# VealFang/PLI-SLAM

Hardware: AMD Instinct MI355X
Metric: stereo frames/sec (ORB+LSD extract+match), 752x480 EuRoC (higher is better)
Workload: dtype u8; 1 GPU; 1xMI355X: 752x480 stereo pairs, extract + stereo Hamming match (BASELINE configs[1] shape, batched); 752x480, 1200 ORB kp (8 levels x1.2) + LSD/LBD (<=100 lines); 256 stereo frames per GPU per step; frames_per_gpu=256, parallelism=frame-batch data parallel, 1 rank(s), gather of result tables to rank 0

## Files before the change

### pli_slam_amd/csrc/common.hpp

```cpp
#pragma once
#include <hip/hip_runtime.h>
#include <cstdint>
#include <cstdio>
#include <cstring>
#include <string>
#include <vector>
#include <map>
#include "../../include/pli_frontend.h"

namespace pli {

constexpr int MAX_LEVELS = 16;
constexpr int CELL_CAP = 512;
constexpr int GRID_COLS = 64;
constexpr int GRID_ROWS = 48;
constexpr int LSD_CHUNK = 4096;

struct LevelGeom {
  int w, h, pitch;
  int64_t offset;
  int minBX, minBY, maxBX, maxBY;
  int nCols, nRows, wCell, hCell;
  int cellBase;
  int nfeatures;
// ... 52 lines not shown
  int races;
  int pad4[31];
};
constexpr int RX_ARENA_BITS = 40;

struct RxSeed {
  int rank, xy;
  float ang, sx, sy;
};

constexpr int RX_QCAP = 16;
constexpr int RX_HAND = RX_QCAP - 8;

struct RxRect {
  int rank, off, cnt;
  float sumdx, sumdy;
  int approx;
};

struct TxDirtyLists {
  int2* list;
  int* cnt;
  const int* order;
  int ts, ntx, nty, W;
  int64_t npix;
  int rmask = -1;
  const int* perm = nullptr;
  int xcdAffine = 0;
  int stamp = 0;
};

constexpr int LSD_ID_INF = 0x7FFFFFFF;
constexpr int TX_EMIT_CAP = 16384;
struct ZeroRanges {
  uint32_t* p[12];
  int64_t words[12];
};

struct TxKeys {
  const double* mg;
  const unsigned long long* maxMg;
  double rho;
  int nBins, pixbits;
  int* idPlane;
  float4* recPack = nullptr;
  int lazyMargin = 8;
  int2* hot = nullptr;
  const float2* cold = nullptr;
  int pack = 0;
};

struct TxTailArgs {
  const DevParams* Pp;
  RxCtl* ctl;
  const float4* rec;
  int2* own;
  const int2* list;
  const int* tileCnt;
  int ts, ntx, nty;
  int* rgSize;
  int2* rgBox;
  int* rgDirty;
  int* tileAct;
  int* tileTouch;
  int TW, TH;
  int* arena;
// ... 37 lines not shown
```

### pli_slam_amd/csrc/kernels.hpp

```cpp
#pragma once
#include "common.hpp"

namespace pli {

struct BlurPlane {
  int w, h, pitchIn, pitchOut;
  int64_t offIn, offOut;
  int tilesX, tileBase;
};
struct BlurJob {
  int nplanes;
  BlurPlane pl[MAX_LEVELS];
  int k[7];
  int radius;
};
struct LbdCoef { float L[21]; float G[63]; };

constexpr signed char ORB_PATTERN_HOST[1024] = {
#include "../../include/pli_orb_pattern.inc"
};
constexpr int orbPatternReach() {
  int best = 0;
  for (int i = 0; i < 512; ++i) {
    const long long x = ORB_PATTERN_HOST[2 * i], y = ORB_PATTERN_HOST[2 * i + 1], r2 = x * x + y * y;
// ... 89 lines not shown
__global__ void k_tri_match(const pli_keypoint* __restrict__ kp1, const uint8_t* __restrict__ desc1, const int* __restrict__ node1, const uint8_t* __restrict__ hasMp1, const uint8_t* __restrict__ stereo1, int n1, const int* __restrict__ kfOff, const pli_keypoint* __restrict__ kfKp, const uint8_t* __restrict__ kfDesc, const uint8_t* __restrict__ kfStereo, const uint32_t* __restrict__ sNode, const uint16_t* __restrict__ sIdx, const int* __restrict__ nListed, const float* __restrict__ F12, const float* __restrict__ ep, const float* __restrict__ scaleFactor, const float* __restrict__ sigma2, int onlyStereo, int coarse, int checkOri, int* __restrict__ matches12, int* __restrict__ stat);
__global__ void k_tri_finish(const pli_keypoint* __restrict__ kp1, int n1, const int* __restrict__ kfOff, const pli_keypoint* __restrict__ kfKp, int* __restrict__ matches12, int* __restrict__ stat);
__global__ void k_kb8_rays(const pli_keypoint* __restrict__ kp1, int n1, int n1Left, const pli_keypoint* __restrict__ kfKp, const int* __restrict__ kfOff, const int* __restrict__ kfNleft, int nkf, Kb8 camL, Kb8 camR, float2* __restrict__ ray1, float2* __restrict__ kfRay);
__global__ void k_tri_match_kb8(const pli_keypoint* __restrict__ kp1, const uint8_t* __restrict__ desc1, const int* __restrict__ node1, const uint8_t* __restrict__ hasMp1, const float2* __restrict__ ray1, int n1, int n1Left, const int* __restrict__ kfOff, const int* __restrict__ kfNleft, const pli_keypoint* __restrict__ kfKp, const uint8_t* __restrict__ kfDesc, const float2* __restrict__ kfRay, const uint32_t* __restrict__ sNode, const uint16_t* __restrict__ sIdx, const int* __restrict__ nListed, const float* __restrict__ rel, Kb8 camL, Kb8 camR, const float* __restrict__ sigma2, int coarse, int checkOri, int* __restrict__ matches12, int* __restrict__ stat);
__global__ void k_search_by_bow_kf(const uint8_t* __restrict__ desc1, const float* __restrict__ angle1, const int* __restrict__ node1, const uint8_t* __restrict__ valid1, int n1, const int* __restrict__ kfOff, const uint8_t* __restrict__ kfDesc, const float* __restrict__ kfAngle, const uint32_t* __restrict__ sNode, const uint16_t* __restrict__ sIdx, const int* __restrict__ nListed, int keyCap, float nnratio, int checkOri, int* __restrict__ matches12, int* __restrict__ nmatchesOut);
struct FuseSurvivor { int kf, mp; float u, v, ur, radius; int level, pad; };
__global__ void k_fuse_grid(const int* __restrict__ kfOff, const pli_keypoint* __restrict__ kfKp, pli_fuse_camera cam, int* __restrict__ cellStart, uint16_t* __restrict__ sIdx);
__global__ void k_fuse_project(const pli_fuse_point* __restrict__ mp, int nmp, int nkf, const float* __restrict__ kfPose, const uint8_t* __restrict__ skip, pli_fuse_camera cam, float th, const float* __restrict__ levelRatio, int nlevels, const float* __restrict__ scaleFactor, FuseSurvivor* __restrict__ surv, int* __restrict__ nSurv, int* __restrict__ bestIdx, int* __restrict__ bestDist);
template <int G> __global__ void k_fuse_match(const FuseSurvivor* __restrict__ surv, const int* __restrict__ nSurv, int nmp, const uint8_t* __restrict__ mpDesc, const int* __restrict__ kfOff, const pli_keypoint* __restrict__ kfKp, const uint8_t* __restrict__ kfDesc, const float* __restrict__ kfUright, const int* __restrict__ cellStart, const uint16_t* __restrict__ sIdx, pli_fuse_camera cam, const float* __restrict__ invSigma2, int reprojGate, int* __restrict__ bestIdx, int* __restrict__ bestDist);
__global__ void k_sim3_project(const pli_fuse_point* __restrict__ mp, int nmp, int npair, const float* __restrict__ kfPose, const uint8_t* __restrict__ skip, pli_fuse_camera cam, float th, const float* __restrict__ levelRatio, int nlevels, const float* __restrict__ scaleFactor, int form, FuseSurvivor* __restrict__ surv, int* __restrict__ candCount, int* __restrict__ bestIdx);
__global__ void k_sim3_candidates(const FuseSurvivor* __restrict__ surv, int64_t nslot, const uint8_t* __restrict__ mpDesc, const int* __restrict__ kfOff, const pli_keypoint* __restrict__ kfKp, const uint8_t* __restrict__ kfDesc, const int* __restrict__ cellStart, const uint16_t* __restrict__ sIdx, pli_fuse_camera cam, int distLimit, int width, unsigned long long* __restrict__ candKeys, int* __restrict__ candCount);
__global__ void k_sim3_assign(const FuseSurvivor* __restrict__ surv, int nmp, const uint8_t* __restrict__ mpDesc, const int* __restrict__ kfOff, const pli_keypoint* __restrict__ kfKp, const uint8_t* __restrict__ kfDesc, const uint8_t* __restrict__ occupied, const int* __restrict__ cellStart, const uint16_t* __restrict__ sIdx, pli_fuse_camera cam, int distLimit, int width, const unsigned long long* __restrict__ candKeys, const int* __restrict__ candCount, int* __restrict__ rowPoint, int* __restrict__ bestIdx, int* __restrict__ nmatchesOut);
__global__ void k_reloc_project(const pli_fuse_point* __restrict__ mp, const int* __restrict__ mpOff, int ncand, const float* __restrict__ pose, pli_fuse_camera cam, float th, const float* __restrict__ levelRatio, int nlevels, const float* __restrict__ scaleFactor, FuseSurvivor* __restrict__ surv, int* __restrict__ candCount, int* __restrict__ bestIdx);
__global__ void k_reloc_candidates(const FuseSurvivor* __restrict__ surv, int64_t nslot, const uint8_t* __restrict__ mpDesc, const int* __restrict__ fOff, const pli_keypoint* __restrict__ fKp, const uint8_t* __restrict__ fDesc, const int* __restrict__ cellStart, const uint16_t* __restrict__ sIdx, pli_fuse_camera cam, int distLimit, int width, unsigned long long* __restrict__ candKeys, int* __restrict__ candCount);
__global__ void k_reloc_assign(const FuseSurvivor* __restrict__ surv, const int* __restrict__ mpOff, const uint8_t* __restrict__ mpDesc, const float* __restrict__ mpAngle, const int* __restrict__ fOff, const pli_keypoint* __restrict__ fKp, const uint8_t* __restrict__ fDesc, int nf, const uint8_t* __restrict__ occupied, const int* __restrict__ cellStart, const uint16_t* __restrict__ sIdx, pli_fuse_camera cam, int distLimit, int width, int checkOri, const unsigned long long* __restrict__ candKeys, const int* __restrict__ candCount, int* __restrict__ rowPoint, int* __restrict__ bestIdx, int* __restrict__ nmatchesOut);
__global__ void k_init_candidates(const pli_keypoint* __restrict__ kp1, const uint8_t* __restrict__ desc1, int n1, const float* __restrict__ prevMatched, const pli_keypoint* __restrict__ kp2, const uint8_t* __restrict__ desc2, const int* __restrict__ cellStart, const uint16_t* __restrict__ sIdx, pli_fuse_camera cam, float radius, int distLimit, int width, unsigned long long* __restrict__ candKeys, int* __restrict__ candCount);
__global__ void k_init_assign(const pli_keypoint* __restrict__ kp1, const uint8_t* __restrict__ desc1, int n1, const float* __restrict__ prevMatched, const pli_keypoint* __restrict__ kp2, const uint8_t* __restrict__ desc2, int n2, const int* __restrict__ cellStart, const uint16_t* __restrict__ sIdx, pli_fuse_camera cam, float radius, int distLimit, int width, float nnratio, int checkOri, const unsigned long long* __restrict__ candKeys, const int* __restrict__ candCount, int* __restrict__ matches12, int* __restrict__ raw12, int* __restrict__ nmatchesOut);
__global__ void k_fisheye_triangulate(const pli_keypoint* __restrict__ kpL, const pli_keypoint* __restrict__ kpR, const int* __restrict__ knnIdx, const int* __restrict__ knnDist, int nl, int nr, int monoL, int monoR, Kb8 c1, Kb8 c2, const float* __restrict__ R12t12, const float* __restrict__ sigma2, int* __restrict__ l2r, int* __restrict__ r2l, float* __restrict__ depth, float* __restrict__ p3d, int* __restrict__ nmatches);
__global__ void k_fill_f32(float* __restrict__ dst, int n, float v);
__global__ void k_proj_assign_fisheye(const pli_proj_query* __restrict__ qL, const pli_proj_query* __restrict__ qR, const uint8_t* __restrict__ qdesc, int nq, const pli_keypoint* __restrict__ kpL, const uint8_t* __restrict__ descL, const uint8_t* __restrict__ occL, const int* __restrict__ l2r, int nL, const pli_keypoint* __restrict__ kpR, const uint8_t* __restrict__ descR, const uint8_t* __restrict__ occR, const int* __restrict__ r2l, int nR, const float* __restrict__ noUright, float minX, float maxX, float minY, float maxY, float nnratio, const unsigned long long* __restrict__ keysL, const int* __restrict__ cntL, const unsigned long long* __restrict__ keysR, const int* __restrict__ cntR, int* __restrict__ mpL, int* __restrict__ mpR, int* __restrict__ nmatchesOut);
__global__ void k_proj2_candidates(const pli_proj_query* __restrict__ q, const uint8_t* __restrict__ qdesc, int nq, const pli_keypoint* __restrict__ kpL, const uint8_t* __restrict__ descL, int nL, const pli_keypoint* __restrict__ kpR, const uint8_t* __restrict__ descR, int nR, const float* __restrict__ noUright, float minX, float maxX, float minY, float maxY, unsigned long long* __restrict__ candKeys, int* __restrict__ candCount, int* __restrict__ leftOpen);
__global__ void k_proj2_assign(const pli_proj_query* __restrict__ q, const uint8_t* __restrict__ qdesc, int nq, const pli_keypoint* __restrict__ kpL, const uint8_t* __restrict__ descL, const uint8_t* __restrict__ occL, int nL, const pli_keypoint* __restrict__ kpR, const uint8_t* __restrict__ descR, const uint8_t* __restrict__ occR, int nR, const float* __restrict__ noUright, float minX, float maxX, float minY, float maxY, int checkOri, const unsigned long long* __restrict__ candKeys, const int* __restrict__ candCount, const int* __restrict__ leftOpen, int* __restrict__ rawIdx2, int* __restrict__ hist, int* __restrict__ accepts);
__global__ void k_proj2_finish(const pli_proj_query* __restrict__ q, int nq, const pli_keypoint* __restrict__ kpL, const pli_keypoint* __restrict__ kpR, int checkOri, const int* __restrict__ rawIdx2, const int* __restrict__ hist, const int* __restrict__ accepts, int* __restrict__ bestIdx2, int* __restrict__ nmatchesOut);
__global__ void k_lapping_order(const pli_keypoint* __restrict__ srcKp, const uint8_t* __restrict__ srcDesc, int n, float lap0, float lap1, pli_keypoint* __restrict__ dstKp, uint8_t* __restrict__ dstDesc, int* __restrict__ monoCount);

__global__ void k_tx_tail(TxTailArgs A);
__global__ void k_tx_rec_from_hot(const RxCtl* __restrict__ ctl, const int2* __restrict__ hotAll, const float2* __restrict__ coldAll, float4* __restrict__ recAll, int64_t npix, int img0);
__global__ void k_tx_hot_trig_err(unsigned long long* __restrict__ maxErrBits);
__global__ void k_tx_cells(RxCtl* __restrict__ ctl, const int* __restrict__ stampAll, int* __restrict__ tileTouchAll, int ncell, int nimg, int img0, int t, int mode, int* __restrict__ list, int* __restrict__ cnt);
__global__ void k_tx_diffmark_cells(RxCtl* __restrict__ ctl, const int2* __restrict__ ownAll, const int* __restrict__ rankAll, const int2* __restrict__ rgBoxAll, int* __restrict__ rgDirtyAll, int* __restrict__ tileActAll, int W, int H, int TW, int TH, int t, int img0, const int* __restrict__ rgLostAll, TxDirtyLists DL, const int* __restrict__ list, const int* __restrict__ cnt);
__global__ void k_tx_prep_cells(const RxCtl* __restrict__ ctl, int2* __restrict__ ownAll, const int* __restrict__ rankAll, const int* __restrict__ rgDirtyAll, int W, int H, int TW, int TH, int t, int img0, int rmask, const int* __restrict__ list, const int* __restrict__ cnt, int stamp);
__global__ void k_zero_ranges(ZeroRanges Z);
__global__ void k_tx_collect(RxCtl* __restrict__ ctl, const int* __restrict__ idPlaneAll, const int2* __restrict__ ownAll, const int* __restrict__ rgSizeAll, int64_t npix, int minReg, int* __restrict__ candAll, int* __restrict__ candCnt, int img0, int emitCap);
__global__ void k_tx_emit_sorted(const RxCtl* __restrict__ ctl, const int* __restrict__ candAll, const int* __restrict__ candCnt, const float4* __restrict__ rgSegAll, int64_t npix, int rmask, float* __restrict__ segAll, int* __restrict__ nSeg, int maxSeg, int img0, int emitCap);
__global__ void k_tx_order(const int* __restrict__ tileCntAll, int ntile, int nimg, int img0, int* __restrict__ perm);
}
```

### pli_slam_amd/csrc/lsd_tile.hip

```cpp
#include "kernels.hpp"
#include "device_prims.hpp"
#include "lsd_rect.hpp"
#include <climits>
#include <type_traits>

namespace pli {

constexpr float TX_NOTDEF = -1024.f;
constexpr int TX_INF = LSD_ID_INF;
constexpr double TX_PI = 3.14159265358979323846;
constexpr double TX_DEG2RAD = TX_PI / 180;
constexpr double TX_3_2_PI = (3 * TX_PI) / 2;
constexpr double TX_2PI = 2 * TX_PI;
#if !defined(PLI_DEV) && (defined(TX_CLAIM_SCOPE) || defined(TX_GROUP) || defined(TX_OWN_LOAD) || defined(TX_DIAG_PAD) || defined(TX_DIAG_NOWAIT) || defined(TX_DIAG_HOT_NOFOLD))
#error "diagnostic builds of lsd_tile.hip need -DPLI_DEV"
#endif
#ifndef TX_CLAIM_SCOPE
#define TX_CLAIM_SCOPE __HIP_MEMORY_SCOPE_AGENT
#endif
#ifndef TX_GROUP
#define TX_GROUP 8
#endif
static_assert(TX_GROUP == 0 || TX_GROUP == 2 || TX_GROUP == 4 || TX_GROUP == 8, "a group member is an octet of lanes");
constexpr int TX_GQ = 768;
// ... 1899 lines not shown
    unsigned hits = 0u;
#pragma unroll
    for (int j = 0; j < 16; ++j) hits |= (sz[j] >= minReg ? 1u : 0u) << j;
    while (hits) {
      const int j = __ffs(hits) - 1;
      hits &= hits - 1u;
      const int64_t p = p1 + (j >> 2) * 1024 + tid * 4 + (j & 3);
      const int id = idPlaneAll[base + p];
      if (id == TX_INF || ownAll[base + p].x != id) continue;
      const int at = atomicAdd(&s_n, 1);
      if (at < CAP) s_buf[at] = id;
      else {
        const int g = atomicAdd(&candCnt[img], 1);
        if (g < emitCap) cand[g] = id;
        else c.overflow = 6;
      }
    }
  }
  __syncthreads();
  const int n = min(s_n, CAP);
  if (tid == 0 && n) s_base = atomicAdd(&candCnt[img], n);
  __syncthreads();
  for (int i = tid; i < n; i += 256) {
    if (s_base + i < emitCap) cand[s_base + i] = s_buf[i];
    else c.overflow = 6;
  }
}

template <int KPT>
__device__ __forceinline__ void tx_emit_sort(unsigned* ks, const int* __restrict__ cand, int n, int tid) {
  unsigned key[KPT];
#pragma unroll
  for (int u = 0; u < KPT; ++u) key[u] = tid * KPT + u < n ? (unsigned)cand[tid * KPT + u] : 0xFFFFFFFFu;
  tx_bitonic_regs<KPT, 1024>(key, ks, tid);
  __syncthreads();
#pragma unroll
  for (int u = 0; u < KPT; ++u) ks[tid * KPT + u] = key[u];
  __syncthreads();
}

__global__ __launch_bounds__(1024) void k_tx_emit_sorted(const RxCtl* __restrict__ ctl, const int* __restrict__ candAll, const int* __restrict__ candCnt,
                                                         const float4* __restrict__ rgSegAll, int64_t npix, int rmask, float* __restrict__ segAll,
                                                         int* __restrict__ nSeg, int maxSeg, int img0, int emitCap) {
  extern __shared__ unsigned ks[];
  const int img = blockIdx.x + img0;
  if (ctl[img].state != 2 || ctl[img].overflow) return;
  const int n = min(candCnt[img], emitCap), tid = threadIdx.x;
  const int* cand = candAll + (int64_t)img * TX_EMIT_CAP;
  if (n <= 1024) tx_emit_sort<1>(ks, cand, n, tid);
  else if (n <= 2048) tx_emit_sort<2>(ks, cand, n, tid);
  else if (n <= 4096) tx_emit_sort<4>(ks, cand, n, tid);
  else if (n <= 8192) tx_emit_sort<8>(ks, cand, n, tid);
  else tx_emit_sort<16>(ks, cand, n, tid);
  float* seg = segAll + (int64_t)img * maxSeg * 4;
  for (int i = tid; i < min(n, maxSeg); i += 1024) {
    const float4 v = rgSegAll[img * npix + (int)(ks[i] & (unsigned)rmask)];
    seg[4 * i + 0] = v.x; seg[4 * i + 1] = v.y; seg[4 * i + 2] = v.z; seg[4 * i + 3] = v.w;
  }
  if (tid == 0) nSeg[img] = min(n, maxSeg);
}

__device__ __forceinline__ bool tx_grid_barrier(unsigned* bar, unsigned target) {
  __shared__ int s_ok;
  asm volatile("s_waitcnt vmcnt(0) lgkmcnt(0)" ::: "memory");
  __syncthreads();
  if (threadIdx.x == 0) {
    __builtin_amdgcn_fence(__ATOMIC_RELEASE, "agent");
    __hip_atomic_fetch_add(&bar[0], 1u, __ATOMIC_RELAXED, __HIP_MEMORY_SCOPE_AGENT);
    int ok = 1;
    unsigned spins = 0;
    while (__hip_atomic_load(&bar[0], __ATOMIC_RELAXED, __HIP_MEMORY_SCOPE_AGENT) < target) {
      __builtin_amdgcn_s_sleep(4);
      if ((++spins & 63u) == 0u &&
          (__hip_atomic_load(&bar[32], __ATOMIC_RELAXED, __HIP_MEMORY_SCOPE_AGENT) != 0u || spins > (1u << 21))) {
        __hip_atomic_store(&bar[32], 1u, __ATOMIC_RELAXED, __HIP_MEMORY_SCOPE_AGENT);
        ok = 0;
        break;
      }
    }
    __builtin_amdgcn_fence(__ATOMIC_ACQUIRE, "agent");
    s_ok = ok;
  }
  __syncthreads();
  asm volatile("s_dcache_inv" ::: "memory");
  return s_ok != 0;
}

__global__ __launch_bounds__(256) void k_tx_tail(TxTailArgs A) {
  __shared__ int qs[4][TX_GQ];
  __shared__ int gbs[4][TX_BMAXBLK + 4];
  __shared__ int parks[4][TX_PARK];
  __shared__ double sts[4][3][64];
  __shared__ double wcs[4][RX_RECT_CACHE][64];
// ... 131 lines not shown
```

### pli_slam_amd/csrc/pli_capi.hip

```cpp
#include "kernels.hpp"
#include "scratch_plan.hpp"
#include <cmath>
#include <cfloat>
#include <algorithm>
#include <memory>
#include <limits>
#include <cstdlib>
#include <set>
#include <string>
#include <functional>
#include <mutex>
#include <atomic>
#include <dlfcn.h>

using namespace pli;

#ifdef PLI_DEV
#define DEVENV(name) getenv(name)
#else
static inline const char* pli_no_devenv() { return nullptr; }
#define DEVENV(name) (pli_no_devenv())
#endif

namespace {
// ... 600 lines not shown
      if (lane || arenaFactor <= 3) return as;
      (void)hipGetLastError();
      arenaFactor = std::max<size_t>(3, arenaFactor / 2);
    }
    c->arenaFactor = (int)arenaFactor;
    if (!lane && arenaFactor < 16 && arenaAsked >= arenaFactor && !DEVENV("PLI_RX_ARENA")) {
      static std::atomic<bool> warned{false};
      if (!warned.exchange(true))
        std::fprintf(stderr, "pli_frontend: the LSD relaxation's arena of this context holds %d words per scaled pixel (16 wanted: %zu images, "
                             "free device memory); results are unchanged, batches of long parallel structures may take the slow fallback "
                             "(pli_lsd_arena_words)\n", (int)arenaFactor, NR);
    }
    if (tiles) {
      c->txTs = (int64_t)NI * ((P.LW + 63) / 64) * ((P.LH + 63) / 64) <= TX_SMALL_TILE_WAVES ? 32 : 64;
      if (const char* e = DEVENV("PLI_TX_TS")) c->txTs = atoi(e) == 16 ? 16 : atoi(e) == 32 ? 32 : atoi(e) == 128 ? 128 : 64;
      c->txNtx = (P.LW + c->txTs - 1) / c->txTs; c->txNty = (P.LH + c->txTs - 1) / c->txTs;
      A(c->txList, (size_t)c->txNtx * c->txNty * c->txTs * c->txTs * NR);
      A(c->txTileCnt, (size_t)c->txNtx * c->txNty * NR);
      A(c->txDirtyList, (size_t)c->txNtx * c->txNty * c->txTs * c->txTs * NR);
      A(c->txDirtyCnt, (size_t)c->txNtx * c->txNty * NR);
      A(c->tailBar, 64);
      A(c->txCellList, (size_t)c->tilesW * c->tilesH * NR);
      A(c->txCellCnt, (size_t)2 * TX_CELL_ROUNDS * NR);
      A(c->txPerm, (size_t)c->txNtx * c->txNty * NR);
      c->txPixBits = 1;
      while (((size_t)1 << c->txPixBits) < npix) ++c->txPixBits;
      int binBits = 1;
      while ((1 << binBits) < P.nBins) ++binBits;
      c->txKeys = c->lsdF64 && P.nBins <= 1024 && (binBits + c->txPixBits < 31 || (binBits + c->txPixBits == 31 && npix < ((size_t)1 << c->txPixBits))) &&
                  !(DEVENV("PLI_TX_KEYS") && atoi(DEVENV("PLI_TX_KEYS")) == 0);
      if (c->txKeys) {
        A(c->txCand, (size_t)TX_EMIT_CAP * NR);
        A(c->txCandCnt, NR);
        HIPCHK(hipFuncSetAttribute(reinterpret_cast<const void*>(k_tx_emit_sorted), hipFuncAttributeMaxDynamicSharedMemorySize, TX_EMIT_CAP * 4));
      }
    }
  }
  A(c->jrCtl, NI);
  c->jrHost.resize(NI);

  A(c->maxG2, NI);
  c->nChunks = (int)((npix + LSD_CHUNK - 1) / LSD_CHUNK);
  A(c->chunkHist, (size_t)NI * c->nChunks * P.nBins);
  A(c->chunkBase, (size_t)NI * c->nChunks * P.nBins);
  if (c->nChunks > 256 && !DEVENV("PLI_LSD_SCAN1")) {
    c->scanChunksPerGroup = 64;
    c->scanGroups = (c->nChunks + c->scanChunksPerGroup - 1) / c->scanChunksPerGroup;
    A(c->scanGroupOff, (size_t)NI * c->scanGroups * P.nBins);
  }
  A(c->nDefined, NI);
  A(c->order, npix * NI);
  A(c->regScratch, npix * NI);
  c->maxSeg = (int)(npix / std::max(P.minRegSize, 1)) + 64;
  A(c->seg, (size_t)NI * c->maxSeg * 4);
  A(c->rectItems, (size_t)NI * c->maxSeg);
  if (c->lsdF64) A(c->rectW, npix * NI);
  A(c->nSeg, NI);
  A(c->tmpKL, (size_t)NI * P.maxLines);
  A(c->dxy, (size_t)P.W * P.H * NI);
  {
    LbdCoef C;
    const int widthOfBand = 7, NUM_OF_BANDS = 9;
    double u = (widthOfBand * 3 - 1) / 2;
    double sigma = (widthOfBand * 2 + 1) / 2;
    double invsigma2 = -1 / (2 * sigma * sigma);
    for (int i = 0; i < widthOfBand * 3; i++) { double dis = i - u; C.L[i] = (float)std::exp(dis * dis * invsigma2); }
    u = (NUM_OF_BANDS * widthOfBand - 1) / 2;
// ... 558 lines not shown
        if (t >= 2)
          TRL(c, "k_rx_classify", k_rx_classify, raster, dim3(256), 0, c->jrCtl, c->own, c->rankOf, c->rgBox,
                 c->rgClean, c->tileMin, P.LW, P.LH, c->tilesW, c->tilesH, t, img0);
        TRL(c, "k_rx_seed", k_rx_seed, dim3((P.LW + 1023) / 1024, P.LH, nimg), dim3(1024), 0, c->jrCtl, c->own, c->rankOf, c->rec, c->lastSize,
               c->rgClean, c->smallSeeds, c->bigSeeds, c->bigCap, P.LW, P.LH, bigThresh, t, img0);
      }
      TRL(c, "k_rx_grow", k_rx_grow, dim3(growBlocks, nimg), dim3(256), 0, c->dP, c->jrCtl, c->rec, c->own, c->smallSeeds,
             c->lastSize, c->rgBox, c->hand, c->handCap, c->arena, c->arenaCap, c->rects, c->rectCap, img0, t);
      if (nimg <= 4)
        TRL(c, "k_rx_grow_wave", k_rx_grow_wave, dim3(bigBlocks * 4, nimg), dim3(64), 0, c->dP, c->jrCtl, c->rec, c->own, c->bigSeeds,
            c->bigCap, c->hand, c->handCap, c->lastSize, c->rgBox, c->arena, c->arenaCap, c->rects, c->rectCap, img0, t);
      else
        TRL(c, "k_rx_grow_big", k_rx_grow_big, dim3(bigBlocks, nimg), dim3(64), 0, c->dP, c->jrCtl, c->rec, c->own, c->bigSeeds,
            c->bigCap, c->hand, c->handCap, c->lastSize, c->rgBox, c->arena, c->arenaCap, c->rects, c->rectCap, img0, t);
      TRL(c, "k_rx_rect", k_rx_rect, dim3(rectBlocks, nimg), dim3(64), 0, c->dP, c->jrCtl, c->rec, c->arena, c->arenaCap, c->rects,
          c->rectCap, c->rgSeg, img0, c->mg, -1, (const int2*)nullptr, (const float2*)nullptr);
      if (trace) {
        HIPCHK(hipMemcpyAsync(c->jrHost.data(), c->jrCtl + img0, sizeof(RxCtl) * nimg, hipMemcpyDeviceToHost, c->stream));
        HIPCHK(hipStreamSynchronize(c->stream));
        const RxCtl& h = c->jrHost[0];
        std::fprintf(stderr, "[rx] t=%d state=%d changed=%d overflow=%d small=%d big=%d hand=%d nextBig=%d rect=%d arena=%lld races=%d\n", t,
                     h.state, h.changed, h.overflow, h.nSmall, h.nBig, h.nHand, h.nextBig, (int)(h.rectArena >> RX_ARENA_BITS),
                     (long long)(h.rectArena & ((1ull << RX_ARENA_BITS) - 1ull)), h.races);
      }
      { pli_status ls_ = look(t); if (ls_ != PLI_OK) return ls_; }
    }
#endif
    }
    if (keyMode) {
      int emitCap = TX_EMIT_CAP;
      if (const char* e = DEVENV("PLI_TX_EMITCAP")) emitCap = std::max(1, std::min(TX_EMIT_CAP, atoi(e)));
      TRL(c, "k_tx_collect", k_tx_collect, dim3(std::max(1, std::min(64, (int)((npix64 + 2047) / 2048))), nimg), dim3(256), 0, c->jrCtl,
          (const int*)c->rankOf, (const int2*)c->own, (const int*)c->lastSize, npix64, P.minRegSize, c->txCand, c->txCandCnt, img0, emitCap);
      TRL(c, "k_tx_emit_sorted", k_tx_emit_sorted, dim3(nimg), dim3(1024), TX_EMIT_CAP * 4, (const RxCtl*)c->jrCtl, (const int*)c->txCand,
          (const int*)c->txCandCnt, (const float4*)c->rgSeg, npix64, (1 << c->txPixBits) - 1, c->seg, c->nSeg, c->maxSeg, img0, emitCap);
      pli_status os = orderPasses(c->jrCtl);
      if (os != PLI_OK) return os;
    } else {
    TRL(c, "k_rx_count", k_rx_count, dim3(c->rxChunks, nimg), dim3(256), 0, c->jrCtl, c->order, c->nDefined, c->own, c->lastSize,
           c->rxChunkCnt, c->rxChunks, npix64, P.minRegSize, img0);
    TRL(c, "k_rx_emit", k_rx_emit, dim3(c->rxChunks, nimg), dim3(256), 0, c->jrCtl, c->order, c->nDefined, c->own, c->lastSize,
           c->rgSeg, c->rxChunkCnt, c->rxChunks, npix64, P.minRegSize, c->seg, c->nSeg, c->maxSeg, img0);
    }
    if (hotAll)
      LAUNCH(c, "k_tx_rec_from_hot", k_tx_rec_from_hot, dim3(std::max(1, std::min(64, (int)((npix64 + 4095) / 4096))), nimg), dim3(256), 0,
             (const RxCtl*)c->jrCtl, (const int2*)c->hot, (const float2*)c->cold, c->rec, npix64, img0);
    if (blocking && !keyMode) {
      for (int i = 0; i < nimg; ++i) {
        if (c->jrHost[i].overflow || c->jrHost[i].state != 2) {
          LAUNCH(c, "k_lsd_grow", k_lsd_grow, dim3(1), dim3(64), 0, c->dP, c->rec, c->mg, c->order, c->nDefined,
                 c->regScratch, c->seg, c->nSeg, c->maxSeg, img0 + i, 1);
        }
      }
    } else {
      LAUNCH(c, "k_lsd_grow_unsettled", k_lsd_grow_unsettled, dim3(nimg), dim3(64), 0, c->dP, c->rec, c->mg, c->order, c->nDefined,
             c->regScratch, c->seg, c->nSeg, c->maxSeg, img0, nimg, c->jrCtl);
      if (!blocking) {
      if (!c->rxSeen) {
        HIPCHK(hipHostMalloc((void**)&c->rxSeen, sizeof(int) * (4 * (size_t)c->NI + 1), hipHostMallocDefault));
        c->rxSeen[4 * (size_t)c->NI] = 0;
        HIPCHK(hipEventCreateWithFlags(&c->evRxSeen, hipEventDisableTiming));
      }
      if (c->rxSeenImages == 0) {
        HIPCHK(hipMemcpy2DAsync(c->rxSeen, 16, c->jrCtl + img0, sizeof(RxCtl), 16, nimg, hipMemcpyDeviceToHost, c->stream));
        if (c->tailBar && c->tailLaunched)
          HIPCHK(hipMemcpyAsync(c->rxSeen + 4 * (size_t)c->NI, c->tailBar + 32, sizeof(int), hipMemcpyDeviceToHost, c->stream));
        else c->rxSeen[4 * (size_t)c->NI] = 0;
        HIPCHK(hipEventRecord(c->evRxSeen, c->stream));
// ... 285 lines not shown
    if (c->rectMap[eye]) { hipFree(c->rectMap[eye]); c->rectMap[eye] = nullptr; }
    return PLI_OK;
  }
  const size_t n = (size_t)c->cfg.width * c->cfg.height;
  if (!c->rectMap[eye]) HIPCHK(hipMalloc(&c->rectMap[eye], n * sizeof(float2)));
  std::vector<float2> h(n);
  for (size_t i = 0; i < n; ++i) h[i] = make_float2(mapx[i], mapy[i]);
  HIPCHK(hipMemcpy(c->rectMap[eye], h.data(), n * sizeof(float2), hipMemcpyHostToDevice));
  return PLI_OK;
}

pli_status pli_ctx_sync(pli_ctx* c) {
  CtxGuard guard__(c);
  if (!c) return PLI_ERR_INVALID;
  HIPCHK(hipStreamSynchronize(c->stream));
  return PLI_OK;
}

pli_status pli_batch_run(pli_ctx* c, int32_t nframes, const uint8_t* dl, const uint8_t* dr, int64_t stride,
                         int64_t frameStride, uint32_t stages, void* table) {
  CtxGuard guard__(c);
  TraceRange range__("pli_batch_run");
  if (!c || !dl || !dr || !table) { g_err = "null argument"; return PLI_ERR_INVALID; }
  if (nframes < 1 || nframes > c->cfg.max_frames) { g_err = "nframes exceeds the context's max_frames"; return PLI_ERR_INVALID; }
  if (stride < c->cfg.width) { g_err = "stride < width"; return PLI_ERR_INVALID; }
  if (((uintptr_t)table & 15) != 0) { g_err = "the table must be 16-byte aligned"; return PLI_ERR_INVALID; }
  HIPCHK(hipSetDevice(c->device));
  uint8_t* T = (uint8_t*)table;
  pli_status st;
  const int nimg = 2 * nframes;
  c->frameFresh = c->pointsFresh = false;
  for (int e = 0; e < 2; ++e) { c->orbDone[e] = c->lineDone[e] = false; c->pyrHostValid[e] = false; }
  if ((st = runIngest(c, dl, dr, stride, frameStride, 0, nimg)) != PLI_OK) return st;
  bool stereoPointsDone = false;
  static const int sideMax = DEVENV("PLI_SIDE_MAX") ? atoi(DEVENV("PLI_SIDE_MAX")) : INT_MAX;
  static const int sideSeqMax = DEVENV("PLI_SIDE_SEQ_MAX") ? atoi(DEVENV("PLI_SIDE_SEQ_MAX")) : 2560;
  const bool seqGrower = c->lsdMode == 2 || (c->lsdMode == 0 && (nimg >= RX_AUTO_IMAGES || nimg > c->rxImages));
  if ((seqGrower ? nimg <= sideSeqMax : nimg < sideMax) && (stages & PLI_RUN_ORB) && (stages & PLI_RUN_LINES) && !c->syncDebug) {
    if (!c->aux) {
      int prLow = 0, prHigh = 0;
      HIPCHK(hipDeviceGetStreamPriorityRange(&prLow, &prHigh));
      if (DEVENV("PLI_SIDE_NOPRIO")) prLow = 0;
      HIPCHK(hipStreamCreateWithPriority(&c->aux, hipStreamNonBlocking, prLow));
      HIPCHK(hipEventCreateWithFlags(&c->evFork, hipEventDisableTiming));
      HIPCHK(hipEventCreateWithFlags(&c->evJoin, hipEventDisableTiming));
      HIPCHK(hipEventCreateWithFlags(&c->evLbdPre, hipEventDisableTiming));
    }
    hipStream_t main = c->stream;
    static const bool sideStereo = DEVENV("PLI_SIDE_NOSTEREO") == nullptr;
    static const bool sideLbd = DEVENV("PLI_SIDE_NOLBD") == nullptr;
    static const bool sideDefer = DEVENV("PLI_SIDE_NODEFER") == nullptr;
    stereoPointsDone = (stages & PLI_RUN_STEREO_POINTS) && sideStereo;
    c->lbdPreOnSide = c->lsdF64 && sideLbd;
    auto sideChain = [c, nimg, nframes, T, stages, main]() -> pli_status {
      HIPCHK(hipEventRecord(c->evFork, main));
      HIPCHK(hipStreamWaitEvent(c->aux, c->evFork, 0));
      c->stream = c->aux;
      pli_status s2 = runOrb(c, 0, nimg, T);
      if (s2 == PLI_OK && (stages & PLI_RUN_STEREO_POINTS) && sideStereo) s2 = runStereoPoints(c, nframes, T);
      if (s2 == PLI_OK && c->lbdPreOnSide) {
        s2 = runLbdPre(c, 0, nimg);
        if (s2 == PLI_OK) { hipError_t e_ = hipEventRecord(c->evLbdPre, c->aux); if (e_ != hipSuccess) s2 = PLI_ERR_HIP; }
      }
      c->stream = main;
      if (s2 != PLI_OK) return s2;
      HIPCHK(hipEventRecord(c->evJoin, c->aux));
      return PLI_OK;
    };
    const int sideDeferMax = DEVENV("PLI_SIDE_DEFER_MAX") ? atoi(DEVENV("PLI_SIDE_DEFER_MAX")) : -1;
    const bool deferSide = sideDeferMax >= 0 ? nimg <= sideDeferMax : (nimg <= 64 || (nimg <= 1024 && (int64_t)c->hp.W * c->hp.H < 500000));
    if (sideDefer && !seqGrower && c->lsdMode != 1 && deferSide) c->sideChain = sideChain;
    else if ((st = sideChain()) != PLI_OK) { c->lbdPreOnSide = false; return st; }
    st = runLines(c, 0, nimg, T);
    if (st == PLI_OK && c->sideChain) { auto f = std::move(c->sideChain); c->sideChain = nullptr; st = f(); }
    c->sideChain = nullptr;
    c->lbdPreOnSide = false;
    if (st != PLI_OK) return st;
    HIPCHK(hipStreamWaitEvent(main, c->evJoin, 0));
  } else {
    if (stages & PLI_RUN_ORB) if ((st = runOrb(c, 0, nimg, T)) != PLI_OK) return st;
    if (stages & PLI_RUN_LINES) if ((st = runLines(c, 0, nimg, T)) != PLI_OK) return st;
  }
  if (stages & PLI_RUN_STEREO_LINES) if ((st = runStereoLines(c, nframes, T)) != PLI_OK) return st;
  if ((stages & PLI_RUN_STEREO_POINTS) && !stereoPointsDone) if ((st = runStereoPoints(c, nframes, T)) != PLI_OK) return st;
  return PLI_OK;
}

pli_status pli_batch_run_host(pli_ctx* c, int32_t nframes, const uint8_t* left, const uint8_t* right, int64_t stride,
                              int64_t frameStride, uint32_t stages, void* table) {
  CtxGuard guard__(c);
  TraceRange range__("pli_batch_run_host");
  if (!c || !left || !right || !table) { g_err = "null argument"; return PLI_ERR_INVALID; }
  if (nframes < 1 || nframes > c->cfg.max_frames) { g_err = "nframes exceeds the context's max_frames"; return PLI_ERR_INVALID; }
  HIPCHK(hipSetDevice(c->device));
  const int W = c->cfg.width, H = c->cfg.height;
  const size_t imgBytes = (size_t)W * H;
  ScratchPlan plan;
  auto dl = plan.add<uint8_t>(2 * imgBytes * nframes);
  auto dt = plan.add<uint8_t>((size_t)c->lay.record_bytes * nframes);
  pli_status st = commitScratch(c, plan);
  if (st != PLI_OK) return st;
  uint8_t* dr = dl + imgBytes * nframes;
  for (int f = 0; f < nframes; ++f) {
    HIPCHK(hipMemcpy2DAsync(dl + imgBytes * f, W, left + (int64_t)f * frameStride, stride, W, H, hipMemcpyHostToDevice, c->stream));
    HIPCHK(hipMemcpy2DAsync(dr + imgBytes * f, W, right + (int64_t)f * frameStride, stride, W, H, hipMemcpyHostToDevice, c->stream));
  }
  HIPCHK(hipMemsetAsync(dt, 0, (size_t)c->lay.record_bytes * nframes, c->stream));
  st = pli_batch_run(c, nframes, dl, dr, W, (int64_t)imgBytes, stages, dt);
  if (st != PLI_OK) return st;
  HIPCHK(hipMemcpyAsync(table, dt, (size_t)c->lay.record_bytes * nframes, hipMemcpyDeviceToHost, c->stream));
  HIPCHK(hipStreamSynchronize(c->stream));
  return PLI_OK;
}

pli_status pli_frame_extract(pli_ctx* c, const uint8_t* left, const uint8_t* right, int32_t w, int32_t h, int64_t strideLeft,
                             int64_t strideRight, void* record) {
// ... 1667 lines not shown
```

Baseline: 6445 stereo frames/s.

## Split LSD segment emit sort into chunked sorts plus merge-rank placement

Replaces the single 1024-thread per-image bitonic sort of line candidates with a two-kernel scheme. The first kernel sorts 1024-element chunks with several 256-thread blocks per image. The second kernel computes each key's global rank by binary-searching every other sorted chunk, then scatters the segment to its final slot. The aim is more parallelism across images and less shared memory per block, at the cost of an extra launch and redundant rank searches when candidate counts are large. The commit also adds env-gated options that move LBD preprocessing within the side stream and launch stereo line matching earlier; both are off by default.

```diff
diff --git a/pli_slam_amd/csrc/common.hpp b/pli_slam_amd/csrc/common.hpp
--- a/pli_slam_amd/csrc/common.hpp
+++ b/pli_slam_amd/csrc/common.hpp
@@ -108,6 +108,7 @@
 
 constexpr int LSD_ID_INF = 0x7FFFFFFF;
 constexpr int TX_EMIT_CAP = 16384;
+constexpr int TX_EMIT_CHUNK = 1024;
 struct ZeroRanges {
   uint32_t* p[12];
   int64_t words[12];
diff --git a/pli_slam_amd/csrc/kernels.hpp b/pli_slam_amd/csrc/kernels.hpp
--- a/pli_slam_amd/csrc/kernels.hpp
+++ b/pli_slam_amd/csrc/kernels.hpp
@@ -145,6 +145,10 @@
 __global__ void k_tx_prep_cells(const RxCtl* __restrict__ ctl, int2* __restrict__ ownAll, const int* __restrict__ rankAll, const int* __restrict__ rgDirtyAll, int W, int H, int TW, int TH, int t, int img0, int rmask, const int* __restrict__ list, const int* __restrict__ cnt, int stamp);
 __global__ void k_zero_ranges(ZeroRanges Z);
 __global__ void k_tx_collect(RxCtl* __restrict__ ctl, const int* __restrict__ idPlaneAll, const int2* __restrict__ ownAll, const int* __restrict__ rgSizeAll, int64_t npix, int minReg, int* __restrict__ candAll, int* __restrict__ candCnt, int img0, int emitCap);
+__global__ void k_tx_emit_chunks(const RxCtl* __restrict__ ctl, int* __restrict__ candAll, const int* __restrict__ candCnt, const float4* __restrict__ rgSegAll, int64_t npix, int rmask, float* __restrict__ segAll, int* __restrict__ nSeg, int maxSeg, int img0, int emitCap);
+__global__ void k_tx_emit_place(const RxCtl* __restrict__ ctl, const int* __restrict__ candAll, const int* __restrict__ candCnt, const float4* __restrict__ rgSegAll, int64_t npix, int rmask, float* __restrict__ segAll, int* __restrict__ nSeg, int maxSeg, int img0, int emitCap);
+#ifdef PLI_DEV
 __global__ void k_tx_emit_sorted(const RxCtl* __restrict__ ctl, const int* __restrict__ candAll, const int* __restrict__ candCnt, const float4* __restrict__ rgSegAll, int64_t npix, int rmask, float* __restrict__ segAll, int* __restrict__ nSeg, int maxSeg, int img0, int emitCap);
+#endif
 __global__ void k_tx_order(const int* __restrict__ tileCntAll, int ntile, int nimg, int img0, int* __restrict__ perm);
 }
diff --git a/pli_slam_amd/csrc/lsd_tile.hip b/pli_slam_amd/csrc/lsd_tile.hip
--- a/pli_slam_amd/csrc/lsd_tile.hip
+++ b/pli_slam_amd/csrc/lsd_tile.hip
@@ -1955,6 +1955,94 @@
   unsigned key[KPT];
 #pragma unroll
   for (int u = 0; u < KPT; ++u) key[u] = tid * KPT + u < n ? (unsigned)cand[tid * KPT + u] : 0xFFFFFFFFu;
+  tx_bitonic_regs<KPT, 256>(key, ks, tid);
+  __syncthreads();
+#pragma unroll
+  for (int u = 0; u < KPT; ++u) ks[tid * KPT + u] = key[u];
+  __syncthreads();
+}
+
+__global__ __launch_bounds__(256) void k_tx_emit_chunks(const RxCtl* __restrict__ ctl, int* __restrict__ candAll, const int* __restrict__ candCnt,
+                                                        const float4* __restrict__ rgSegAll, int64_t npix, int rmask, float* __restrict__ segAll,
+                                                        int* __restrict__ nSeg, int maxSeg, int img0, int emitCap) {
+  extern __shared__ unsigned ks[];
+  const int img = blockIdx.y + img0;
+  if (ctl[img].state != 2 || ctl[img].overflow) return;
+  const int n = min(candCnt[img], emitCap), tid = threadIdx.x, c0 = blockIdx.x * TX_EMIT_CHUNK;
+  if (c0 >= n) {
+    if (blockIdx.x == 0 && tid == 0) nSeg[img] = 0;
+    return;
+  }
+  const int m = min(n - c0, TX_EMIT_CHUNK);
+  int* cand = candAll + (int64_t)img * TX_EMIT_CAP + c0;
+  if (m <= 256) tx_emit_sort<1>(ks, cand, m, tid);
+  else if (m <= 512) tx_emit_sort<2>(ks, cand, m, tid);
+  else tx_emit_sort<4>(ks, cand, m, tid);
+  if (n > TX_EMIT_CHUNK) {
+    for (int i = tid; i < m; i += 256) cand[i] = (int)ks[i];
+    return;
+  }
+  float* seg = segAll + (int64_t)img * maxSeg * 4;
+  for (int i = tid; i < min(n, maxSeg); i += 256) {
+    const float4 v = rgSegAll[img * npix + (int)(ks[i] & (unsigned)rmask)];
+    seg[4 * i + 0] = v.x; seg[4 * i + 1] = v.y; seg[4 * i + 2] = v.z; seg[4 * i + 3] = v.w;
+  }
+  if (tid == 0) nSeg[img] = min(n, maxSeg);
+}
+
+__global__ __launch_bounds__(256) void k_tx_emit_place(const RxCtl* __restrict__ ctl, const int* __restrict__ candAll, const int* __restrict__ candCnt,
+                                                       const float4* __restrict__ rgSegAll, int64_t npix, int rmask, float* __restrict__ segAll,
+                                                       int* __restrict__ nSeg, int maxSeg, int img0, int emitCap) {
+  __shared__ unsigned buf[TX_EMIT_CHUNK];
+  constexpr int KPT = TX_EMIT_CHUNK / 256;
+  const int img = blockIdx.y + img0;
+  if (ctl[img].state != 2 || ctl[img].overflow) return;
+  const int n = min(candCnt[img], emitCap), tid = threadIdx.x, c0 = blockIdx.x * TX_EMIT_CHUNK;
+  if (n <= TX_EMIT_CHUNK || c0 >= n) return;
+  const unsigned* cand = reinterpret_cast<const unsigned*>(candAll + (int64_t)img * TX_EMIT_CAP);
+  const int m = min(n - c0, TX_EMIT_CHUNK);
+  unsigned key[KPT];
+  int at[KPT];
+#pragma unroll
+  for (int u = 0; u < KPT; ++u) {
+    const int i = tid + 256 * u;
+    key[u] = i < m ? cand[c0 + i] : 0xFFFFFFFFu;
+    at[u] = i;
+  }
+  for (int d0 = 0; d0 < n; d0 += TX_EMIT_CHUNK) {
+    if (d0 == c0) continue;
+    const int md = min(n - d0, TX_EMIT_CHUNK);
+    __syncthreads();
+    for (int i = tid; i < TX_EMIT_CHUNK; i += 256) buf[i] = i < md ? cand[d0 + i] : 0xFFFFFFFFu;
+    __syncthreads();
+    int pos[KPT];
+#pragma unroll
+    for (int u = 0; u < KPT; ++u) pos[u] = 0;
+#pragma unroll
+    for (int s = TX_EMIT_CHUNK / 2; s > 0; s >>= 1) {
+#pragma unroll
+      for (int u = 0; u < KPT; ++u) pos[u] += buf[pos[u] + s - 1] < key[u] ? s : 0;
+    }
+#pragma unroll
+    for (int u = 0; u < KPT; ++u) at[u] += pos[u] + (buf[pos[u]] < key[u] ? 1 : 0);
+  }
+  float* seg = segAll + (int64_t)img * maxSeg * 4;
+#pragma unroll
+  for (int u = 0; u < KPT; ++u) {
+    if (tid + 256 * u < m && at[u] < maxSeg) {
+      const float4 v = rgSegAll[img * npix + (int)(key[u] & (unsigned)rmask)];
+      seg[4 * at[u] + 0] = v.x; seg[4 * at[u] + 1] = v.y; seg[4 * at[u] + 2] = v.z; seg[4 * at[u] + 3] = v.w;
+    }
+  }
+  if (blockIdx.x == 0 && tid == 0) nSeg[img] = min(n, maxSeg);
+}
+
+#ifdef PLI_DEV
+template <int KPT>
+__device__ __forceinline__ void tx_emit_sort1k(unsigned* ks, const int* __restrict__ cand, int n, int tid) {
+  unsigned key[KPT];
+#pragma unroll
+  for (int u = 0; u < KPT; ++u) key[u] = tid * KPT + u < n ? (unsigned)cand[tid * KPT + u] : 0xFFFFFFFFu;
   tx_bitonic_regs<KPT, 1024>(key, ks, tid);
   __syncthreads();
 #pragma unroll
@@ -1970,11 +2058,11 @@
   if (ctl[img].state != 2 || ctl[img].overflow) return;
   const int n = min(candCnt[img], emitCap), tid = threadIdx.x;
   const int* cand = candAll + (int64_t)img * TX_EMIT_CAP;
-  if (n <= 1024) tx_emit_sort<1>(ks, cand, n, tid);
-  else if (n <= 2048) tx_emit_sort<2>(ks, cand, n, tid);
-  else if (n <= 4096) tx_emit_sort<4>(ks, cand, n, tid);
-  else if (n <= 8192) tx_emit_sort<8>(ks, cand, n, tid);
-  else tx_emit_sort<16>(ks, cand, n, tid);
+  if (n <= 1024) tx_emit_sort1k<1>(ks, cand, n, tid);
+  else if (n <= 2048) tx_emit_sort1k<2>(ks, cand, n, tid);
+  else if (n <= 4096) tx_emit_sort1k<4>(ks, cand, n, tid);
+  else if (n <= 8192) tx_emit_sort1k<8>(ks, cand, n, tid);
+  else tx_emit_sort1k<16>(ks, cand, n, tid);
   float* seg = segAll + (int64_t)img * maxSeg * 4;
   for (int i = tid; i < min(n, maxSeg); i += 1024) {
     const float4 v = rgSegAll[img * npix + (int)(ks[i] & (unsigned)rmask)];
@@ -1982,6 +2070,7 @@
   }
   if (tid == 0) nSeg[img] = min(n, maxSeg);
 }
+#endif
 
 __device__ __forceinline__ bool tx_grid_barrier(unsigned* bar, unsigned target) {
   __shared__ int s_ok;
diff --git a/pli_slam_amd/csrc/pli_capi.hip b/pli_slam_amd/csrc/pli_capi.hip
--- a/pli_slam_amd/csrc/pli_capi.hip
+++ b/pli_slam_amd/csrc/pli_capi.hip
@@ -656,7 +656,9 @@
       if (c->txKeys) {
         A(c->txCand, (size_t)TX_EMIT_CAP * NR);
         A(c->txCandCnt, NR);
+#ifdef PLI_DEV
         HIPCHK(hipFuncSetAttribute(reinterpret_cast<const void*>(k_tx_emit_sorted), hipFuncAttributeMaxDynamicSharedMemorySize, TX_EMIT_CAP * 4));
+#endif
       }
     }
   }
@@ -1281,8 +1283,19 @@
       if (const char* e = DEVENV("PLI_TX_EMITCAP")) emitCap = std::max(1, std::min(TX_EMIT_CAP, atoi(e)));
       TRL(c, "k_tx_collect", k_tx_collect, dim3(std::max(1, std::min(64, (int)((npix64 + 2047) / 2048))), nimg), dim3(256), 0, c->jrCtl,
           (const int*)c->rankOf, (const int2*)c->own, (const int*)c->lastSize, npix64, P.minRegSize, c->txCand, c->txCandCnt, img0, emitCap);
-      TRL(c, "k_tx_emit_sorted", k_tx_emit_sorted, dim3(nimg), dim3(1024), TX_EMIT_CAP * 4, (const RxCtl*)c->jrCtl, (const int*)c->txCand,
-          (const int*)c->txCandCnt, (const float4*)c->rgSeg, npix64, (1 << c->txPixBits) - 1, c->seg, c->nSeg, c->maxSeg, img0, emitCap);
+#ifdef PLI_DEV
+      if (DEVENV("PLI_TAIL_EMIT1K"))
+        TRL(c, "k_tx_emit_sorted", k_tx_emit_sorted, dim3(nimg), dim3(1024), TX_EMIT_CAP * 4, (const RxCtl*)c->jrCtl, (const int*)c->txCand,
+            (const int*)c->txCandCnt, (const float4*)c->rgSeg, npix64, (1 << c->txPixBits) - 1, c->seg, c->nSeg, c->maxSeg, img0, emitCap);
+      else
+#endif
+      {
+        const dim3 chunks((emitCap + TX_EMIT_CHUNK - 1) / TX_EMIT_CHUNK, nimg);
+        TRL(c, "k_tx_emit_chunks", k_tx_emit_chunks, chunks, dim3(256), TX_EMIT_CHUNK * 4, (const RxCtl*)c->jrCtl, c->txCand,
+            (const int*)c->txCandCnt, (const float4*)c->rgSeg, npix64, (1 << c->txPixBits) - 1, c->seg, c->nSeg, c->maxSeg, img0, emitCap);
+        TRL(c, "k_tx_emit_place", k_tx_emit_place, chunks, dim3(256), 0, (const RxCtl*)c->jrCtl, (const int*)c->txCand,
+            (const int*)c->txCandCnt, (const float4*)c->rgSeg, npix64, (1 << c->txPixBits) - 1, c->seg, c->nSeg, c->maxSeg, img0, emitCap);
+      }
       pli_status os = orderPasses(c->jrCtl);
       if (os != PLI_OK) return os;
     } else {
@@ -1634,7 +1647,7 @@
   c->frameFresh = c->pointsFresh = false;
   for (int e = 0; e < 2; ++e) { c->orbDone[e] = c->lineDone[e] = false; c->pyrHostValid[e] = false; }
   if ((st = runIngest(c, dl, dr, stride, frameStride, 0, nimg)) != PLI_OK) return st;
-  bool stereoPointsDone = false;
+  bool stereoPointsDone = false, stereoLinesDone = false;
   static const int sideMax = DEVENV("PLI_SIDE_MAX") ? atoi(DEVENV("PLI_SIDE_MAX")) : INT_MAX;
   static const int sideSeqMax = DEVENV("PLI_SIDE_SEQ_MAX") ? atoi(DEVENV("PLI_SIDE_SEQ_MAX")) : 2560;
   const bool seqGrower = c->lsdMode == 2 || (c->lsdMode == 0 && (nimg >= RX_AUTO_IMAGES || nimg > c->rxImages));
@@ -1653,17 +1666,23 @@
     static const bool sideLbd = DEVENV("PLI_SIDE_NOLBD") == nullptr;
     static const bool sideDefer = DEVENV("PLI_SIDE_NODEFER") == nullptr;
     stereoPointsDone = (stages & PLI_RUN_STEREO_POINTS) && sideStereo;
-    c->lbdPreOnSide = c->lsdF64 && sideLbd;
-    auto sideChain = [c, nimg, nframes, T, stages, main]() -> pli_status {
+    const int lbdPreAt = DEVENV("PLI_TAIL_LBDPRE") ? atoi(DEVENV("PLI_TAIL_LBDPRE")) : 0;
+    c->lbdPreOnSide = c->lsdF64 && sideLbd && lbdPreAt != 3;
+    auto sideChain = [c, nimg, nframes, T, stages, main, lbdPreAt]() -> pli_status {
       HIPCHK(hipEventRecord(c->evFork, main));
       HIPCHK(hipStreamWaitEvent(c->aux, c->evFork, 0));
       c->stream = c->aux;
-      pli_status s2 = runOrb(c, 0, nimg, T);
+      pli_status s2 = PLI_OK;
+      auto lbdPre = [&](int at) {
+        if (s2 != PLI_OK || !c->lbdPreOnSide || at != lbdPreAt) return;
+        s2 = runLbdPre(c, 0, nimg);
+        if (s2 == PLI_OK && hipEventRecord(c->evLbdPre, c->aux) != hipSuccess) s2 = PLI_ERR_HIP;
+      };
+      lbdPre(1);
+      if (s2 == PLI_OK) s2 = runOrb(c, 0, nimg, T);
+      lbdPre(2);
       if (s2 == PLI_OK && (stages & PLI_RUN_STEREO_POINTS) && sideStereo) s2 = runStereoPoints(c, nframes, T);
-      if (s2 == PLI_OK && c->lbdPreOnSide) {
-        s2 = runLbdPre(c, 0, nimg);
-        if (s2 == PLI_OK) { hipError_t e_ = hipEventRecord(c->evLbdPre, c->aux); if (e_ != hipSuccess) s2 = PLI_ERR_HIP; }
-      }
+      lbdPre(0);
       c->stream = main;
       if (s2 != PLI_OK) return s2;
       HIPCHK(hipEventRecord(c->evJoin, c->aux));
@@ -1678,12 +1697,14 @@
     c->sideChain = nullptr;
     c->lbdPreOnSide = false;
     if (st != PLI_OK) return st;
+    if ((stages & PLI_RUN_STEREO_LINES) && DEVENV("PLI_TAIL_STEREO_LINES_EARLY")) { st = runStereoLines(c, nframes, T); stereoLinesDone = true; }
     HIPCHK(hipStreamWaitEvent(main, c->evJoin, 0));
+    if (st != PLI_OK) return st;
   } else {
     if (stages & PLI_RUN_ORB) if ((st = runOrb(c, 0, nimg, T)) != PLI_OK) return st;
     if (stages & PLI_RUN_LINES) if ((st = runLines(c, 0, nimg, T)) != PLI_OK) return st;
   }
-  if (stages & PLI_RUN_STEREO_LINES) if ((st = runStereoLines(c, nframes, T)) != PLI_OK) return st;
+  if ((stages & PLI_RUN_STEREO_LINES) && !stereoLinesDone) if ((st = runStereoLines(c, nframes, T)) != PLI_OK) return st;
   if ((stages & PLI_RUN_STEREO_POINTS) && !stereoPointsDone) if ((st = runStereoPoints(c, nframes, T)) != PLI_OK) return st;
   return PLI_OK;
 }
```

Result: no change. 6401 stereo frames/s (-0.7%).
